# jvstinian/libzombsole

Hardware: AMD Instinct MI355X
Metric: env-steps/sec (whole node), 65 536 parallel 64×64 envs at 1/2/4/8 MI355X (higher is better)
Workload: dtype int32

## Files before the change

### libzombsole_amd/csrc/engine.hip

```cpp
#include <hip/hip_runtime.h>

#include <algorithm>
#include <cstdio>
#include <cstring>
#include <string>
#include <vector>

#include "zs_launch.hpp"
#include "zs_obs_state.hpp"
#include "zs_snapshot.hpp"
#include "zs_record.hpp"
#include "zs_mask.hpp"
#include "zs_entity_obs.hpp"
#include "zs_entity_act.hpp"
#include "zs_autopilot.hpp"
#include "zs_episode.hpp"

static thread_local std::string g_err;

static int fail(int code, const std::string& msg) {
    g_err = msg;
    return code;
}

// ... 10 lines not shown
    do {                                                                                       \
        hipError_t _e = (x);                                                                   \
        if (_e != hipSuccess) return fail(ZS_EHIP, std::string(#x ": ") + hipGetErrorString(_e)); \
    } while (0)

#define TRY(x)             \
    do {                   \
        int _r = (x);      \
        if (_r) return _r; \
    } while (0)

static int launched(const char* name, hipError_t e) {
    return e == hipSuccess ? ZS_OK : fail(ZS_EHIP, std::string(name) + ": " + hipGetErrorString(e));
}
#define LAUNCHCHK(name, x) TRY(launched((name), (x)))

struct zs_handle {
    zs_config cfg;
    zs_launch ov;
    int device;
    Dev d;
    ObsPlan obs;
    StepPlan step;
    struct GraphSet {
        hipGraphExec_t g[2] = {nullptr, nullptr};
        const void* key[9] = {};
        uint64_t used = 0;
    };
    static const int kGraphSets = 4;
    GraphSet gsets[kGraphSets];
    uint64_t gclock = 0;
    bool graphs_stale = false;
    uint64_t* d_gstep = nullptr;
    int graph_pol = 0;
    int reset_side = 0;
    hipStream_t s_reset = nullptr;
    hipEvent_t ev_rfork = nullptr, ev_rjoin = nullptr;
    int state_words;
    std::vector<void*> allocs;
    int32_t* d_state;
    uint64_t* d_seedbuf;
    int* d_err;
    int* d_rlist[2];
    int* d_rcount;
    int rpar = 0;
    uint64_t snap_fp = 0;
    int32_t* d_envp_owner = nullptr;
    void* mask_bound = nullptr;
    int32_t* d_obj_xy = nullptr;
    void* ent_bound = nullptr;
    int ent_kz = 0, ent_kp = 0;
    const int32_t* eact_ids = nullptr;
    void* eact_mask = nullptr;
    int eact_kz = 0, eact_kp = 0;
    NavPlan nav{};
    void* nav_bound = nullptr;
    int nav_fields = 0, nav_max_dist = 0;
    const uint8_t* pilot_policy = nullptr;
    int32_t* pilot_out = nullptr;
    const char* step_last = "";
    EpisodeArgs ep{};
    uint8_t* d_ep_reset = nullptr;
    RenderArgs rn{};
    HostLayout hl{};
    int32_t* h_hin = nullptr;
    int32_t* d_hin = nullptr;
    int32_t* h_hrec = nullptr;
// ... 495 lines not shown
    std::vector<uint64_t> seeds(N);
    for (size_t i = 0; i < N; i++) seeds[i] = i;
    TRY(seed_envs(h, 0, (int)N, seeds.data(), nullptr));
    hipError_t se = hipDeviceSynchronize();
    if (se != hipSuccess) return fail(ZS_EHIP, std::string("zs_create sync: ") + hipGetErrorString(se));
    *out = h;
    owner.h = nullptr;
    return ZS_OK;
}

extern "C" int zs_obs_shape(const zs_handle* h, int32_t out[4]) {
    if (!h || !out) return fail(ZS_EINVAL, "null argument");
    const Dev& d = h->d;
    bool world = d.obs_scope == ZS_OBS_WORLD;
    out[0] = world ? 1 : (d.reward_mode == ZS_REWARD_MULTI ? d.A : 1);
    out[1] = d.obs_enc == ZS_ENC_CHANNELS ? 3 : 1;
    out[2] = world ? d.H : d.obs_w;
    out[3] = world ? d.W : d.obs_w;
    return ZS_OK;
}

extern "C" int zs_seed(zs_handle* h, int32_t env0, int32_t n, const uint64_t* seeds_host, void* stream) {
    if (!h || !seeds_host) return fail(ZS_EINVAL, "null argument");
    NOT_ON_VIEWER(h, "zs_seed");
    return seed_envs(h, env0, n, seeds_host, stream);
}

static int seed_envs(zs_handle* h, int32_t env0, int32_t n, const uint64_t* seeds_host, void* stream) {
    if (env0 < 0 || n < 0 || env0 + n > h->d.N) return fail(ZS_EINVAL, "env range out of bounds");
    if (n == 0) return ZS_OK;
    ENTER(h, stream, s);
    HIPCHK(hipMemcpyAsync(h->d_seedbuf, seeds_host, sizeof(uint64_t) * n, hipMemcpyHostToDevice, s));
    HIPCHK(launch_seed(s, h->d, env0, n, h->d_seedbuf));
    HIPCHK(hipStreamSynchronize(s));
    return ZS_OK;
}

struct TickUnit {
    decltype(&launch_tick_g1) launch;
    decltype(&stamps_g1) stamps;
};
static const TickUnit& tick_unit(int G) {
#define ZS_UNIT(g) {launch_tick_g##g, stamps_g##g}
    static const TickUnit units[7] = {ZS_UNIT(1), ZS_UNIT(2), ZS_UNIT(4), ZS_UNIT(8), ZS_UNIT(16), ZS_UNIT(32), ZS_UNIT(64)};
#undef ZS_UNIT
    return units[__builtin_ctz((unsigned)G)];
}

static int launch_obs(zs_handle* h, const Dev& d, void* obs, const uint8_t* mask, hipStream_t s, int env0 = 0, int env1 = -1) {
    if (!obs) return ZS_OK;
    if (env1 < 0) env1 = d.N;
    const ObsKernel& k = mask ? h->obs.masked : h->obs.full;
    const ObsLaunch o = {k, obs_grid(k, env1 - env0), obs, mask, env0, env1};
    return timed_launch(h, s, h->ev_obs, "observation launch", [&] { return obs_launch(d.obs_dtype, o, s, d); });
}

static int launch_tick(zs_handle* h, const Dev& d, const int32_t* actions, double* rew, uint8_t* done, uint8_t* trunc,
                       uint8_t* listed, uint8_t* reset_out, int* rlist, int* rcount, void* obs, hipStream_t s,
                       int env0 = 0, int env1 = -1) {
    const StepPlan& sp = h->step;
    const int ne = 64 / sp.G;
    if (env1 < 0) env1 = d.N;
    unsigned grid = (unsigned)((env1 - env0 + ne - 1) / ne);
    const int p = h->rpar;
    const TickArgs a = {actions, rew,  done, trunc,      listed,        reset_out,       rlist,   rcount,
                        obs,     env0, env1, sp.n_reset, h->d_rlist[p], h->d_rcount + p, h->d_err};
// ... 31 lines not shown
        }
    }
    if (h->ep.run) HIPCHK(launch_episode_clear(s, h->ep, env_mask_dev, 1));
    if (h->rn.body_col) HIPCHK(launch_render_track(s, h->rn, env_mask_dev, 1));
    return launch_obs(h, h->d, obs_dev, env_mask_dev, s);
}

extern "C" int zs_reset(zs_handle* h, const uint8_t* env_mask_dev, void* obs_dev, void* stream) {
    if (!h) return fail(ZS_EINVAL, "null handle");
    NOT_ON_VIEWER(h, "zs_reset");
    ENTER(h, stream, s);
    TRY(queue_reset(h, env_mask_dev, obs_dev, s));
    int err;
    TRY(read_error_word(h, s, &err));
    return reset_result(err);
}

extern "C" int zs_observe(zs_handle* h, const uint8_t* env_mask_dev, void* obs_dev, void* stream) {
    if (!h || !obs_dev) return fail(ZS_EINVAL, "null argument");
    ENTER(h, stream, s);
    return launch_obs(h, h->d, obs_dev, env_mask_dev, s);
}

extern "C" int zs_step(zs_handle* h, const int32_t* actions_dev, void* obs_dev, double* rewards_dev, uint8_t* done_dev,
                       uint8_t* trunc_dev, uint8_t* listed_dev, uint8_t* reset_dev, void* stream) {
    if (!h || !actions_dev || !rewards_dev || !done_dev || !trunc_dev) return fail(ZS_EINVAL, "null argument");
    NOT_ON_VIEWER(h, "zs_step");
    ENTER(h, stream, s);
    if ((h->ep.run || h->rn.body_col) && !reset_dev) reset_dev = h->d_ep_reset;
    if (h->eact_ids)
        LAUNCHCHK("k_entity_act_decode",
                  launch_entity_act_decode(s, h->d, h->eact_kz, h->eact_kp, nullptr, h->eact_ids, const_cast<int32_t*>(actions_dev)));
    int q = 1 - h->rpar, rc = ZS_OK;
    bool side = false;
    if (!h->step.fused) {
        side = h->reset_side != 0;
        hipStream_t rs = s;
        if (side) {
            HIPCHK(hipEventRecord(h->ev_rfork, s));
            HIPCHK(hipStreamWaitEvent(h->s_reset, h->ev_rfork, 0));
            rs = h->s_reset;
        }
        if (h->graph_pol && side)
            HIPCHK(launch_gen_actions_ctr(s, h->d, (const uint64_t*)h->d_gstep, h->graph_pol, (int32_t*)actions_dev));
        TRY(launch_reset(h, h->d, 1, nullptr, h->d.fobs ? obs_dev : nullptr, rs));
        if (side) HIPCHK(hipEventRecord(h->ev_rjoin, h->s_reset));
    }
    Dev d = h->d;
    d.pol_n = side ? 0 : h->graph_pol;
    d.pol_step = side ? nullptr : h->d_gstep;
    const int p = h->rpar;
    TRY(launch_tick(h, d, actions_dev, rewards_dev, done_dev, trunc_dev, listed_dev, reset_dev, h->d_rlist[q],
                    h->d_rcount + q, obs_dev, s));
    h->rpar = q;
    auto tail_on_error = [&](int code) {
        hipStreamCaptureStatus cs = hipStreamCaptureStatusNone;
        if (hipStreamIsCapturing(s, &cs) == hipSuccess && cs == hipStreamCaptureStatusNone) {
            (void)hipMemsetAsync(h->d_rcount + p, 0, sizeof(int), s);
            if (h->d.defer_respawn) (void)hipMemsetAsync(h->d.resp_count, 0, sizeof(int), s);
        }
        return code;
    };
    if (h->d.defer_respawn) {
        rc = launch_respawn(h, d, s);
        if (rc) return tail_on_error(rc);
    }
    if (side && hipStreamWaitEvent(s, h->ev_rjoin, 0) != hipSuccess) return tail_on_error(fail(ZS_EHIP, "hipStreamWaitEvent"));
    d.tail_cnt0 = h->d_rcount + p;
    d.tail_cnt1 = d.defer_respawn ? d.resp_count : nullptr;
    d.tail_step = h->graph_pol ? h->d_gstep : nullptr;
    if (d.fobs || !obs_dev) {
        rc = launched("k_tail", launch_tail(s, d));
        if (rc) return tail_on_error(rc);
        h->step_last = "k_tail";
    } else {
        rc = launch_obs(h, d, obs_dev, nullptr, s);
        if (rc) return tail_on_error(rc);
        h->step_last = obs_kernel_name(h->obs.full.kind);
    }
    if (h->mask_bound) LAUNCHCHK("k_action_mask", launch_action_mask(s, d, nullptr, h->mask_bound));
    if (h->ent_bound) {
        const EntityArgs g = {h->ent_kz, h->ent_kp, d.nobj, h->d_obj_xy};
        LAUNCHCHK("k_entity_obs", launch_entity_obs(s, d, g, nullptr, h->ent_bound));
    }
    if (h->eact_mask) LAUNCHCHK("k_entity_act_mask", launch_entity_act_mask(s, d, h->eact_kz, h->eact_kp, nullptr, h->eact_mask));
    if (h->nav_bound) {
// ... 260 lines not shown
extern "C" int zs_step_graph_n(zs_handle* h, uint64_t step0, int32_t n_discrete, int32_t n_steps, int32_t* actions_dev,
                               void* obs_dev, double* rewards_dev, uint8_t* done_dev, uint8_t* trunc_dev,
                               uint8_t* listed_dev, uint8_t* reset_dev, void* stream) {
    if (!h || !actions_dev || !rewards_dev || !done_dev || !trunc_dev) return fail(ZS_EINVAL, "null argument");
    NOT_ON_VIEWER(h, "zs_step_graph");
    if (n_discrete < 0 || n_discrete > 7) return fail(ZS_EINVAL, "n_discrete must be in 0..7");
    if (n_steps < 1 || n_steps > 64) return fail(ZS_EINVAL, "n_steps must be in 1..64");
    if (n_discrete != 0 && h->eact_ids)
        return fail(ZS_EINVAL, "zs_step_graph: n_discrete must be 0 while entity-action ids are bound (the generated policy "
                               "would overwrite the decoded rows)");
    ENTER(h, stream, s);
    if (h->graphs_stale) {
        HIPCHK(hipStreamSynchronize(s));
        for (auto& gs : h->gsets) {
            HIPCHK(destroy_graphs(gs));
            gs.used = 0;
        }
        h->graphs_stale = false;
    }
    const void* key[9] = {actions_dev, obs_dev, rewards_dev, done_dev, trunc_dev, listed_dev, reset_dev,
                          (const void*)(intptr_t)n_discrete, (const void*)(intptr_t)n_steps};
    zs_handle::GraphSet* set = nullptr;
    for (auto& gs : h->gsets) {
        bool same = gs.g[0] && gs.g[1];
        for (int k = 0; k < 9 && same; k++) same = key[k] == gs.key[k];
        if (same) set = &gs;
    }
    if (!set) {
        set = &h->gsets[0];
        for (auto& gs : h->gsets)
            if (gs.used < set->used) set = &gs;
        HIPCHK(destroy_graphs(*set));
        if (!h->d_gstep) {
            TRY(dalloc(h, &h->d_gstep, 2));
        }
        uint64_t init[2] = {step0, 0};
        if (n_discrete > 0) HIPCHK(hipMemcpyAsync(h->d_gstep, init, sizeof(init), hipMemcpyHostToDevice, s));
        HIPCHK(hipStreamSynchronize(s));
        hipStream_t cs;
        HIPCHK(hipStreamCreateWithFlags(&cs, hipStreamNonBlocking));
        const int prof = h->prof;
        h->prof = 0;
        const int p0 = h->rpar;
        int rc = ZS_OK;
        for (int g = 0; g < 2 && rc == ZS_OK; g++) {
            hipGraph_t graph = nullptr;
            h->rpar = (p0 + g) & 1;
            if (hipStreamBeginCapture(cs, hipStreamCaptureModeThreadLocal) != hipSuccess) {
                rc = fail(ZS_EHIP, "hipStreamBeginCapture failed");
                break;
            }
            h->graph_pol = n_discrete;
            for (int k = 0; k < n_steps && rc == ZS_OK; k++)
                rc = zs_step(h, actions_dev, obs_dev, rewards_dev, done_dev, trunc_dev, listed_dev, reset_dev, cs);
            h->graph_pol = 0;
            hipError_t ce = hipStreamEndCapture(cs, &graph);
            if (rc == ZS_OK && ce != hipSuccess) rc = fail(ZS_EHIP, std::string("hipStreamEndCapture: ") + hipGetErrorString(ce));
            if (rc == ZS_OK) {
                hipError_t ie = hipGraphInstantiate(&set->g[(p0 + g) & 1], graph, nullptr, nullptr, 0);
                if (ie != hipSuccess) rc = fail(ZS_EHIP, std::string("hipGraphInstantiate: ") + hipGetErrorString(ie));
            }
            if (graph) (void)hipGraphDestroy(graph);
        }
        h->rpar = p0;
        h->prof = prof;
        (void)hipStreamDestroy(cs);
        if (rc != ZS_OK) {
            (void)destroy_graphs(*set);
            return rc;
        }
// ... 296 lines not shown

extern "C" int zs_profile_read(zs_handle* h, double* out) {
    if (!h || !out) return fail(ZS_EINVAL, "null argument");
    HIPCHK(hipSetDevice(h->device));
    double tot[4] = {0.0, 0.0, 0.0, 0.0};
    EventList* lists[4] = {&h->ev_tick, &h->ev_obs, &h->ev_reset, &h->ev_respawn};
    for (int k = 0; k < 4; k++)
        for (auto& pr : *lists[k]) {
            HIPCHK(hipEventSynchronize(h->ev_pool[pr.second]));
            float ms = 0.f;
            HIPCHK(hipEventElapsedTime(&ms, h->ev_pool[pr.first], h->ev_pool[pr.second]));
            tot[k] += ms;
        }
    for (int k = 0; k < 4; k++) out[2 * k] = tot[k], out[2 * k + 1] = (double)lists[k]->size();
    prof_clear(h);
    return ZS_OK;
}

extern "C" int zs_describe(zs_handle* h, char* buf, int32_t len) {
    if (!h || !buf || len <= 0) return fail(ZS_EINVAL, "null argument");
    const Dev& d = h->d;
    const ObsKernel& kf = h->obs.full;
    const StepPlan& p = h->step;
    snprintf(buf, (size_t)len,
             "{\"envs\": %d, \"entities\": %d, \"lanes_per_env\": %d, \"step_kernel\": \"%s\", \"step_lds\": %d, "
             "\"step_wgs_per_cu\": %d, \"rng_window\": %d, \"obs_kernel\": \"%s\", \"reset_side_stream\": %d, "
             "\"reset_lds\": %d, \"respawn\": \"%s\", \"tick_waves\": %d, \"rng_step\": %d, \"par_exec\": %d, "
             "\"obs_kernel_masked\": \"%s\", \"obs_encoders\": \"%s\", \"mask_kernel\": \"k_action_mask\", "
             "\"mask_grid\": %u, \"mask_block\": %d, \"mask_bound\": %d, \"env_params\": %d, \"episode_stats\": %d, "
             "\"render\": %d, \"render_grid\": %d, \"render_block\": %d, \"entity_obs_bound\": %d, \"entity_kz\": %d, "
             "\"entity_kp\": %d, \"autopilot_kernel\": \"k_autopilot\", \"autopilot_grid\": %u, \"autopilot_block\": %d, "
             "\"autopilot_bound\": %d, \"nav_bound\": %d, \"nav_fields\": %d, \"nav_max_dist\": %d, \"nav_kernel\": \"k_nav\", "
             "\"nav_envs_per_wg\": %d, \"nav_block\": %d, \"nav_lds_bytes\": %d, \"entity_act_kernel\": \"k_entity_act\", "
             "\"entity_act_ids_bound\": %d, \"entity_act_mask_bound\": %d, \"step_tail_launch\": \"%s\"}",
             d.N, d.E, p.G, p.fused ? "k_step" : "k_tick", p.lds, p.resident, p.rw_cap,
             d.fobs ? "step launch" : obs_kernel_name(kf.kind), h->reset_side,
             p.reset_lds, p.defer_respawn ? "k_respawn" : "tick", p.tick_waves, p.rw_step,
             d.par_exec, obs_kernel_name(h->obs.masked.kind), obs_encoders_name(kf), zs_mask_grid(d.N), ZS_MASK_BLOCK,
             h->mask_bound ? 1 : 0, (d.flags & ZS_FLAG_ENV_PARAMS) ? 1 : 0, h->ep.run ? 1 : 0, h->rn.body_col ? 1 : 0,
             h->rn.body_col ? h->rn.plan.bands : 0, h->rn.body_col ? ZS_RENDER_BLOCK : 0,
             h->ent_bound ? 1 : 0, h->ent_kz, h->ent_kp, zs_pilot_grid(d.N), ZS_PILOT_BLOCK, h->pilot_out ? 1 : 0,
             h->nav_bound ? 1 : 0, h->nav_fields, h->nav_max_dist, h->nav.envs_per_wg, h->nav.block, h->nav.lds_bytes,
             h->eact_ids ? 1 : 0, h->eact_mask ? 1 : 0, h->step_last);
    return ZS_OK;
}

static int read_log(zs_handle* h, const int32_t* log, const int32_t* log_n, int words, int lo, int32_t env, int32_t* out_host,
                    int32_t cap, int32_t* n_out, void* stream) {
    if (!h || !n_out || (cap > 0 && !out_host)) return fail(ZS_EINVAL, "null argument");
    if (!log) return fail(ZS_EINVAL, "the handle was created without ZS_FLAG_DEATH_LOG");
    if (env < 0 || env >= h->d.N) return fail(ZS_EINVAL, "env out of range");
    ENTER(h, stream, s);
    int32_t n = 0;
    HIPCHK(hipMemcpyAsync(&n, log_n + env, sizeof(int32_t), hipMemcpyDeviceToHost, s));
    HIPCHK(hipStreamSynchronize(s));
    n = std::max(lo, std::min(n, h->d.E));
    const int k = std::min(n < 0 ? -1 - n : n, std::max(0, (int)cap));
    if (k > 0) {
        HIPCHK(hipMemcpyAsync(out_host, log + (size_t)env * h->d.E * words, sizeof(int32_t) * words * k, hipMemcpyDeviceToHost, s));
        HIPCHK(hipStreamSynchronize(s));
    }
    *n_out = n;
    return ZS_OK;
}

extern "C" int zs_action_log(zs_handle* h, int32_t env, int32_t* out_host, int32_t cap, int32_t* n_out, void* stream) {
    return read_log(h, h ? h->d.alog : nullptr, h ? h->d.alog_n : nullptr, 2, h ? -1 - h->d.E : 0, env, out_host, cap, n_out, stream);
}

extern "C" int zs_death_log(zs_handle* h, int32_t env, int32_t* out_host, int32_t cap, int32_t* n_out, void* stream) {
    return read_log(h, h ? h->d.dlog : nullptr, h ? h->d.dlog_n : nullptr, 5, 0, env, out_host, cap, n_out, stream);
}

static int obs_bytes_per_env(const zs_handle* h) {
    int32_t shp[4];
    zs_obs_shape(h, shp);
// ... 178 lines not shown
```

### libzombsole_amd/csrc/zs_device.hpp

```cpp
#pragma once
#include <hip/hip_runtime.h>
#include <stdint.h>

#include "../../include/zombsole_mi355x.h"
#include "zs_obs_plan.hpp"
#include "zs_step_plan.hpp"

#ifndef ZS_RESET_WAVES
#define ZS_RESET_WAVES 3
#endif

#define ZS_MT_M 397
#define ZS_RING_WORDS (2 * ZS_MT_N)

#define EIX(d, s, e) ((size_t)(e) * (d).E + (s))

enum {
    S_T = 0,
    S_DEATHS,
    S_ZD,
    S_EPSTEPS,
    S_NORDER,
    S_NEEDRESET,
    S_PREVZD,
// ... 32 lines not shown
    const int32_t* zspawn;
    const int32_t* agent_weapons;
    const int32_t* agent_codes;
    const int32_t* bot_types;
    int32_t* pos;
    int32_t* life;
    uint8_t* weapon;
    uint8_t* present;
    uint32_t* serial;
    uint8_t* order;
    int32_t* scal;
    int32_t* prev_life;
    uint8_t* listed;
    int32_t* obst_hp;
    uint32_t* hp_dirty;
    const int32_t* hp_init;
    int hp_chunk;
    uint32_t hp_chunk_m;
    uint32_t hp_chunk_m32;
    uint32_t* dead_dirty;
    const uint32_t* dead_zero;
    int dead_chunk;
    uint32_t dead_chunk_m;
    uint32_t dead_chunk_m32;
    const uint32_t* opres_full;
    uint32_t w_m;
    uint32_t* obst_present;
    uint32_t* obst_nonpos;
    uint32_t* dead;
    uint32_t* ring;
    uint32_t* rngst;
    const uint64_t* pol_step;
    int pol_n;
    int* tail_cnt0;
    int* tail_cnt1;
    uint64_t* tail_step;
    uint64_t* seeds;
    int32_t* cand;
    int* resp_list;
    int* resp_count;
    int32_t* dlog;
    int32_t* dlog_n;
    int32_t* alog;
    int32_t* alog_n;
    uint32_t* ovf;
};

#define SC_OBST_MASK 0xffffu
#define SC_KIND_SHIFT 16
#define SC_OBJ_BIT (1u << 20)
#define OPAD_OBJ 8u

#ifdef ZS_STAMPS
#define ZS_NPHASE 28
#define ZS_STAMP_WGS 65536
#endif

enum { EP_INITIAL = 0, EP_MINIMUM, EP_MAXSTEPS, EP_N };
__host__ __device__ __forceinline__ int32_t* envp_cur(const Dev& d) { return d.scal + (size_t)S_NSCAL * d.N; }
__host__ __device__ __forceinline__ int32_t* envp_next(const Dev& d) { return d.scal + (size_t)(S_NSCAL + EP_N) * d.N; }

__device__ __forceinline__ const Dev* zs_launder_dev(const Dev& d0) {
    typedef const __attribute__((address_space(4))) Dev CDev;
    CDev* dp = (CDev*)__builtin_amdgcn_kernarg_segment_ptr();
    asm volatile("" : "+s"(dp));
#ifdef ZS_CHECK_LAUNDER
    if (dp->N != d0.N || dp->E != d0.E || dp->pos != d0.pos || dp->ring != d0.ring) __builtin_trap();
#else
    (void)d0;
#endif
    return (const Dev*)dp;
}

#define ZS_HP_FLOOR (-2147483647)

__device__ __forceinline__ int32_t hp_store_value(const Dev& d, int64_t v) {
    if (v < -32768) {
        uint32_t f = ZS_OVF_INT16;
        if (v < (int64_t)ZS_HP_FLOOR) {
            v = ZS_HP_FLOOR;
            f |= ZS_OVF_INT32;
        }
        if ((__hip_atomic_load(d.ovf, __ATOMIC_RELAXED, __HIP_MEMORY_SCOPE_AGENT) & f) != f) atomicOr(d.ovf, f);
    }
    return (int32_t)v;
}

__device__ __forceinline__ void step_tail(const Dev& d) {
    if (d.tail_cnt0) *d.tail_cnt0 = 0;
    if (d.tail_cnt1) *d.tail_cnt1 = 0;
    if (d.tail_step) *d.tail_step += 1;
}

__device__ __forceinline__ uint64_t splitmix64(uint64_t x) {
    uint64_t z = x + 0x9E3779B97F4A7C15ull;
    z = (z ^ (z >> 30)) * 0xBF58476D1CE4E5B9ull;
    z = (z ^ (z >> 27)) * 0x94D049BB133111EBull;
    return z ^ (z >> 31);
}

static __constant__ int32_t c_discrete[7][3] = {{ZS_ACT_MOVE, 0, 1},  {ZS_ACT_MOVE, -1, 0},       {ZS_ACT_MOVE, 0, -1},
                                         {ZS_ACT_MOVE, 1, 0},  {ZS_ACT_ATTACK_CLOSEST, 0, 0}, {ZS_ACT_HEAL, 0, 0},
                                         {ZS_ACT_HEAL_CLOSEST, 0, 0}};

__device__ __forceinline__ int policy_id(uint64_t seed, uint64_t step, int n, int a) {
    return (int)(splitmix64(splitmix64(splitmix64(seed) ^ step) ^ (uint64_t)a) % (uint64_t)n);
}
__device__ __forceinline__ int32_t policy_action(uint64_t seed, uint64_t step, int n, int k) {
    const int a = k / 3;
    return c_discrete[policy_id(seed, step, n, a)][k - 3 * a];
}

__device__ __forceinline__ int32_t pack_xy(int x, int y) { return (int32_t)((uint32_t)(x & 0xffff) | ((uint32_t)y << 16)); }
__device__ __forceinline__ int unpack_x(int32_t p) { return (int)(int16_t)(p & 0xffff); }
__device__ __forceinline__ int unpack_y(int32_t p) { return (int)(p >> 16); }

__device__ __forceinline__ void wave_sync() {
    __builtin_amdgcn_fence(__ATOMIC_RELEASE, "wavefront");
    __builtin_amdgcn_wave_barrier();
    __builtin_amdgcn_fence(__ATOMIC_ACQUIRE, "wavefront");
}

__device__ __forceinline__ uint32_t mt_temper(uint32_t y) {
    y ^= (y >> 11);
    y ^= (y << 7) & 0x9d2c5680u;
    y ^= (y << 15) & 0xefc60000u;
    y ^= (y >> 18);
    return y;
}

__device__ __forceinline__ uint32_t mt_f(uint32_t a, uint32_t b, uint32_t c) {
    uint32_t y = (a & 0x80000000u) | (b & 0x7fffffffu);
    return c ^ (y >> 1) ^ ((y & 1u) ? 0x9908b0dfu : 0u);
}

__device__ inline void mt_twist_serial(uint32_t* dst, const uint32_t* src) {
    for (int i = 0; i < ZS_MT_N; i++) {
        uint32_t b = (i + 1 < ZS_MT_N) ? src[i + 1] : dst[0];
        uint32_t c = (i + ZS_MT_M < ZS_MT_N) ? src[i + ZS_MT_M] : dst[i + ZS_MT_M - ZS_MT_N];
        dst[i] = mt_f(src[i], b, c);
    }
}

// ... 102 lines not shown
```

### libzombsole_amd/csrc/zs_obs.hpp

```cpp
#pragma once
#include "zs_device.hpp"
#include "zs_obs_plan.hpp"

typedef unsigned int zs_v4u __attribute__((ext_vector_type(4)));
typedef unsigned int zs_v2u __attribute__((ext_vector_type(2)));
typedef int zs_v2i __attribute__((ext_vector_type(2)));
typedef int zs_v4i __attribute__((ext_vector_type(4)));

__device__ __forceinline__ int xcd_remap(int b, int nb) {
    const int q = nb >> 3, r = nb & 7, x = b & 7, k = b >> 3;
    return x * q + (x < r ? x : r) + k;
}

struct XcdDeal {
    int base, span, off, w, ucount;
    __device__ XcdDeal(int b, int nb, int n_units, int W) : w(W) {
        const int q = nb >> 3, r = nb & 7, x = b & 7, j = b >> 3;
        const int gs = x * q + (x < r ? x : r), gx = q + (x < r);
        const int r0 = (int)((long long)n_units * gs / nb), r1 = (int)((long long)n_units * (gs + gx) / nb);
        base = r0;
        span = gx * W;
        off = j * W;
        const int m = r1 - r0 - off;
        ucount = m <= 0 ? 0 : (m / span) * W + min(m % span, W);
// ... 946 lines not shown
    lv4u* st4 = (lv4u*)smem;
    lu8* slots = (lu8*)(smem + stat_bytes + RING_ENC * enc_bytes);
    ZS_LDS int* state = (ZS_LDS int*)(slots + US * SLOT);
    if (threadIdx.x < RING_SLOTS) state[threadIdx.x] = 0;
    if (PATCHED) {
        patch_stage_static(d, smem);
    } else {
        obs_stage_static4(d, st4, threadIdx.x, blockDim.x);
        __syncthreads();
    }
    const int G = gridDim.x, n_units = (env1 - env0 + PAIR - 1) / PAIR;
    const XcdDeal deal(blockIdx.x, G, n_units, RING_WRT);
    const int ucount = deal.ucount;
    auto unit_of = [&](int u) { return deal.unit(u); };
    const int count = ucount ? PAIR * (ucount - 1) + min(PAIR, env1 - env0 - PAIR * unit_of(ucount - 1)) : 0;
    auto unit_env = [&](int u) { return env0 + PAIR * unit_of(u); };
    if (wave >= RING_ENC) {
        for (int u = wave - RING_ENC; u < ucount; u += RING_WRT) {
            const int q = u % US, e = unit_env(u);
            const bool whole = PAIR * u + PAIR <= count;
            for (int h = 0; h < PAIR; h++)
                if (PAIR * u + h < count) ring_wait(&state[PAIR * q + h], 2 * u + 1);
            if (whole) obs_stage_flush<T, NOBS * PAIR, RING_THR>(slots + q * SLOT, out + (size_t)e * BLK, lane);
            else obs_stage_flush<T, NOBS, RING_THR>(slots + q * SLOT, out + (size_t)e * BLK, lane);
            for (int h = 0; h < PAIR; h++) ring_state_store(&state[PAIR * q + h], 2 * u + 2);
        }
        return;
    }
    lu8* img = (lu8*)(smem + stat_bytes + wave * enc_bytes);
    PatchEnc<S> pe(d, smem, img, lane);
    const li32* pos = (const li32*)(img + L.off_pos);
    const int code_s = lane < d.A ? d.agent_codes[lane < d.A ? lane : 0] : (lane < d.A + d.P ? ZS_THING_PLAYER : ZS_THING_ZOMBIE);
    auto item_env = [&](int t) { return unit_env(t / PAIR) + t % PAIR; };
    int t = wave;
    if (t >= count) return;
    auto encode = [&](int t, ObsPrefetch& f, zs_v2u& dq) {
        const Dev& d = *zs_launder_dev(d0);
        const int u = t / PAIR, h = t % PAIR, e = item_env(t);
        if (PATCHED) pe.build(d, f);
        else obs_build_compact(d, L, img, f, code_s, lane);
        const int tn = t + 2 * RING_ENC, tq = t + 4 * RING_ENC;
        obs_prefetch_env(d, item_env(tn < count ? tn : wave), dq, f);
        dq = obs_dirty(d, item_env(tq < count ? tq : wave));
        wave_sync();
        if (!PATCHED) obs_window_compact<NOBS>(d, L, img, lane);
        const int q = u % US;
        if (u >= US) ring_wait(&state[PAIR * q + h], 2 * (u - US) + 2);
        wave_sync();
        ZS_LDS S* ot0 = (ZS_LDS S*)(slots + q * SLOT) + (int)((uintptr_t)(out + (size_t)(e - h) * BLK) & 15) / TS + h * BLK;
#pragma unroll
        for (int a = 0; a < NOBS; a++) {
            if (PATCHED) {
                pe.block(d, ot0 + a * 3 * PLANE, a);
            } else {
                const int32_t ap = pos[a];
                const int ox = unpack_x(ap) - WW / 2, oy = unpack_y(ap) - WW / 2;
                const lu8* wm = img + a * PLANE;
                obs_encode_block<S>(d, L, st4, img, wm, ox, oy, ot0 + a * 3 * PLANE, lane);
            }
        }
        ring_state_store(&state[PAIR * q + h], 2 * u + 1);
    };
    auto envc = [&](int tt) { return item_env(tt < count ? tt : wave); };
    ObsPrefetch fa, fb;
    zs_v2u qa, qb;
    obs_prefetch_env(d, envc(t), OBS_OWN_ROWS, fa);
    obs_prefetch_env(d, envc(t + RING_ENC), obs_dirty(d, envc(t + RING_ENC)), fb);
    qa = obs_dirty(d, envc(t + 2 * RING_ENC));
    qb = obs_dirty(d, envc(t + 3 * RING_ENC));
    for (; t < count; t += 2 * RING_ENC) {
        encode(t, fa, qa);
        if (t + RING_ENC < count) encode(t + RING_ENC, fb, qb);
    }
}

#ifndef BRING_THR
#define BRING_THR RING_THR
#endif
__device__ __forceinline__ uint32_t chunk_of(uint32_t x, uint32_t m32) { return m32 ? __umulhi(x, m32) : x; }


template <typename T, int NOBS>
__global__ void __launch_bounds__(64 * (BRING_ENC + BRING_WRT), 1) k_obs_pbring(Dev d, T* out, int env0, int env1, int us) {
    if (blockIdx.x == 0 && threadIdx.x == 0) step_tail(d);
    extern __shared__ __align__(16) uint8_t smem[];
    typedef typename obs_stage<T>::type S;
    constexpr int WW = 21, PLANE = WW * WW, PER = PLANE / 63, TS = (int)sizeof(T);
    static_assert(PLANE % 63 == 0, "63 lanes x PER rows of three");
    constexpr int PAIR = ring_pair(TS, NOBS), SLOT = obs_stage_slot_bytes(TS, NOBS * PAIR), BLK = NOBS * 3 * PLANE;
    const int wave = __builtin_amdgcn_readfirstlane(threadIdx.x >> 6), lane = threadIdx.x & 63;
    const int encb = pbring_enc_bytes(d.DW, d.OW);
    lv4u* st4 = (lv4u*)smem;
    lu8* slots = (lu8*)(smem + 16 * d.DW + BRING_ENC * encb);
    ZS_LDS int* state = (ZS_LDS int*)(slots + us * SLOT);
    if (threadIdx.x < 8) state[threadIdx.x] = 0;
    obs_stage_static4(d, st4, threadIdx.x, blockDim.x);
    __syncthreads();
    const int G = gridDim.x, n_units = (env1 - env0 + PAIR - 1) / PAIR;
    const XcdDeal deal(blockIdx.x, G, n_units, BRING_WRT);
    const int ucount = deal.ucount;
    const int count = ucount ? PAIR * (ucount - 1) + min(PAIR, env1 - env0 - PAIR * deal.unit(ucount - 1)) : 0;
    auto unit_env = [&](int u) { return env0 + PAIR * deal.unit(u); };
    if (wave >= BRING_ENC) {
        for (int u = wave - BRING_ENC; u < ucount; u += BRING_WRT) {
            const int q = u % us, e = unit_env(u);
            const bool whole = PAIR * u + PAIR <= count;
            for (int h = 0; h < PAIR; h++)
                if (PAIR * u + h < count) ring_wait(&state[PAIR * q + h], 2 * u + 1);
            if (whole) obs_stage_flush<T, NOBS * PAIR, BRING_THR>(slots + q * SLOT, out + (size_t)e * BLK, lane);
            else obs_stage_flush<T, NOBS, BRING_THR>(slots + q * SLOT, out + (size_t)e * BLK, lane);
            for (int h = 0; h < PAIR; h++) ring_state_store(&state[PAIR * q + h], 2 * u + 2);
        }
        return;
    }
    lu32* idead = (lu32*)(smem + 16 * d.DW + wave * encb);
    lu32* iopres = (lu32*)(smem + 16 * d.DW + wave * encb + ((d.DW * 4 + 15) / 16) * 16);
    const int code_s = lane < d.A ? d.agent_codes[lane < d.A ? lane : 0] : (lane < d.A + d.P ? ZS_THING_PLAYER : ZS_THING_ZOMBIE);
    const int W = d.W, H = d.H, sl = lane < d.E ? lane : d.E - 1;
    const int lr = lane / WW, lq = lane - lr * WW;
    auto item_env = [&](int t) { return unit_env(t / PAIR) + t % PAIR; };
    if (wave >= count) return;
    struct R1 {
        int32_t p, l, w, r;
        uint32_t hd, dd;
    };
    struct R23 {
        uint32_t dv[BRING_D], ov[BRING_O];
        int32_t hv[NOBS][PER];
    };
    auto envc = [&](int t) { return item_env(t < count ? t : wave); };
    auto round1 = [&](int t, R1& r) {
        const int e = envc(t);
        r.p = d.pos[EIX(d, sl, e)];
        r.l = d.life[EIX(d, sl, e)];
        r.w = d.weapon[EIX(d, sl, e)];
        r.r = d.present[EIX(d, sl, e)];
        r.hd = d.hp_dirty[e];
        r.dd = d.dead_dirty[e];
    };
    auto round23 = [&](int t, const R1& r, R23& q) {
        const int e = envc(t);
        const uint32_t* dr = d.dead + (size_t)e * d.DW;
#pragma unroll
        for (int i = 0; i < BRING_D; i++) {
            const int w = min(lane + 64 * i, d.DW - 1);
            q.dv[i] = (((r.dd >> chunk_of((uint32_t)w, d.dead_chunk_m32)) & 1u) ? dr : d.dead_zero)[w];
        }
        const uint32_t* orow = r.hd ? d.obst_present + (size_t)e * d.OW : d.opres_full;
#pragma unroll
        for (int i = 0; i < BRING_O; i++) q.ov[i] = orow[min(lane + 64 * i, max(d.OW - 1, 0))];
        const int32_t* hrow = d.obst_hp + (size_t)e * d.O;
#pragma unroll
        for (int a = 0; a < NOBS; a++) {
            const int32_t ap = __builtin_amdgcn_readlane(r.p, a);
// ... 63 lines not shown
#pragma unroll
            for (int a = 0; a < NOBS; a++) {
                const int32_t ap = __builtin_amdgcn_readlane(r.p, a);
                const int dx = x - (unpack_x(ap) - WW / 2), dy = y - (unpack_y(ap) - WW / 2);
                if ((unsigned)dx < (unsigned)WW && (unsigned)dy < (unsigned)WW) {
                    ZS_LDS S* ot = ot0 + a * 3 * PLANE;
                    const int cc = dy * WW + dx;
                    ot[cc] = (S)code_s;
                    ot[PLANE + cc] = obs_val<S>(r.l);
                    ot[2 * PLANE + cc] = (S)r.w;
                }
            }
        }
        ring_state_store(&state[PAIR * qs + h], 2 * u + 1);
        wave_sync();
    };
    R1 ra, rb;
    R23 qa, qb;
    int t = wave;
    round1(t, ra);
    round1(t + BRING_ENC, rb);
    round23(t, ra, qa);
    auto step = [&](int t, R1& rx, R23& qx, R1& ry, R23& qy) {
        build(qx);
        round23(t + BRING_ENC, ry, qy);
        const R1 cur = rx;
        round1(t + 2 * BRING_ENC, rx);
        encode(t, cur, qx);
    };
    for (; t < count; t += 2 * BRING_ENC) {
        step(t, ra, qa, rb, qb);
        if (t + BRING_ENC < count) step(t + BRING_ENC, rb, qb, ra, qa);
    }
}
```

### libzombsole_amd/csrc/zs_tick.hpp

```cpp
#pragma once
#include "zs_device.hpp"
#include "zs_obs.hpp"

#define NOTHING ((int)0x80000000)

enum { K_NONE = 0, K_MOVE = 1, K_ATTACK = 2, K_HEAL = 3, K_DEFER = 4, K_RAISE = 5 };

#ifdef ZS_STAMPS
static __device__ unsigned long long g_stamp_wg[ZS_STAMP_WGS * ZS_NPHASE];
#define STAMP_DECL unsigned long long _st_prev = 0;
#define STAMP(k)                                                                          \
    do {                                                                                  \
        unsigned long long _t;                                                            \
        asm volatile("s_memtime %0\n\ts_waitcnt lgkmcnt(0)" : "=s"(_t)::"memory");      \
        if ((k) > 0 && threadIdx.x == 0 && blockIdx.x < ZS_STAMP_WGS)                     \
            g_stamp_wg[blockIdx.x * ZS_NPHASE + (k)-1] += _t - _st_prev;                  \
        _st_prev = _t;                                                                    \
    } while (0)
#define SUB_DECL unsigned long long _sub_prev;
#define SUB(k)                                                                            \
    do {                                                                                  \
        unsigned long long _t;                                                            \
        asm volatile("s_memtime %0\n\ts_waitcnt lgkmcnt(0)" : "=s"(_t)::"memory");      \
        if ((k) > 0 && blockIdx.x < ZS_STAMP_WGS && c.g == 0)                             \
// ... 1281 lines not shown
    c.lrank = (lu8*)(smem + L.off_rank);
    c.lkind = (lu8*)(smem + L.off_kind);
    c.lperm = (lu8*)(smem + L.off_perm);
    c.lmoved = (lu8*)(smem + L.off_moved);
    c.lact = (li32*)(smem + L.off_act);
    c.xs = (li32*)(smem + L.off_xs);
    c.lists = (li32*)(smem + L.off_lists);
    if (dp->lists_cap)
        for (int i = lane; i < dp->nps + dp->nzs; i += 64) c.lists[i] = i < dp->nps ? dp->pspawn[i] : dp->zspawn[i - dp->nps];

    STAMP_DECL
    STAMP(0);
    int needs_reset = 0, stepping = 0, n_order = 0;
    uint32_t st0 = 0, st = 0;
    int wlen = 0;
    int32_t vp[4], vl[4];
    uint8_t vw[4], vr[4], vo[4];
    int mval = 0, av = 0;
    uint32_t bmv[8], opw = 0u;
    uint32_t wv[4];
    uint64_t pseed = 0, pstep = 0;
    auto window = [&](uint32_t st_, uint32_t& off, uint32_t& slot, uint32_t& ready) {
        off = st_ & 1023u, slot = (st_ >> 10) & 1u, ready = (st_ >> 11) & 1u;
        if (off >= ZS_MT_N && ready) {
            slot ^= 1u;
            off = 0;
            ready = 0;
        }
        const int maxw = off >= ZS_MT_N ? 0 : (ready ? dp->rw_cap : min(dp->rw_cap, ZS_MT_N - (int)off));
        return min(dp->rw_step, maxw);
    };
    const int nmisc = MISC_N + 2 * A;
    int pmin = 0, pmax = 0;
    if (active) {
        if (dp->pol_n) {
            pseed = dp->seeds[e];
            pstep = *dp->pol_step;
        } else if (A) {
            av = actions[(size_t)e * A * 3 + min(j, 3 * A - 1)];
        }
        needs_reset = dp->scal[S_NEEDRESET * N + e];
        n_order = dp->scal[S_NORDER * N + e];
        st = dp->rngst[e];
#pragma unroll
        for (int u = 0; u < 4; u++) {
            const int s = j + u * G;
            if (s < E) {
                vp[u] = dp->pos[EIX(*dp, s, e)];
                vl[u] = dp->life[EIX(*dp, s, e)];
                vw[u] = dp->weapon[EIX(*dp, s, e)];
                vr[u] = dp->present[EIX(*dp, s, e)];
                vo[u] = dp->order[EIX(*dp, s, e)];
            }
        }
        mval = misc_load(*dp, min(j, nmisc - 1), e);
        opw = dp->obst_present[(size_t)e * dp->OW + min(j, max(dp->OW - 1, 0))];
    }
#pragma unroll
    for (int u = 0; u < 8; u++)
        if (64 * u < dp->DW) bmv[u] = dp->obstbits[min(lane + 64 * u, dp->DW - 1)];
    stepping = active && needs_reset == 0;
    if (active && dp->pol_n) {
        for (int k = j; k < 3 * A; k += G) {
            const int32_t v = policy_action(pseed, pstep, dp->pol_n, k);
            ((int32_t*)actions)[(size_t)e * A * 3 + k] = v;
            if (stepping) LACT(c, k) = v;
        }
    }
#pragma unroll
    for (int u = 0; u < 8; u++)
        if (64 * u < dp->DW && lane + 64 * u < dp->DW) bcast_row<NE>(c.bm, lane + 64 * u, bmv[u]);
    for (int w = 512 + lane; w < dp->DW; w += 64) bcast_row<NE>(c.bm, w, dp->obstbits[w]);
    if (stepping) {
#pragma unroll
        for (int u = 0; u < 4; u++) {
            const int s = j + u * G;
            if (s < E) {
                c.lpos[IX(c, s)] = vp[u];
                c.llife[IX(c, s)] = vl[u];
                c.lweap[IX(c, s)] = vw[u];
                c.lpres[IX(c, s)] = vr[u];
                c.lorder[IX(c, s)] = vo[u];
            }
        }
        if (j < nmisc) MISC(c, j) = mval;
        if (!dp->pol_n) {
            if (j < 3 * A) LACT(c, j) = av;
            for (int k = j + G; k < 3 * A; k += G) LACT(c, k) = actions[(size_t)e * A * 3 + k];
        }
        SX(1);
        {
            auto ix = [&](int s) { return IX(c, s); };

            for (int b = j + 4 * G; b < E; b += 4 * G) {
                int32_t vp[4], vl[4];
                uint8_t vw[4], vr[4], vo[4];
#pragma unroll
// ... 253 lines not shown
            dp->order[EIX(*dp, s, e)] = LO(c, s);
        }
        for (int f = j; f < MISC_N + 2 * A; f += G) misc_store(*dp, f, e, MISC(c, f));
    }
    wave_sync();
    STAMP(6);
    ZS_RELOAD_DEV();
    if (dp->fobs && obs_out) {
        const unsigned long long stepmask = __ballot(stepping && leader);
        lu8* img = (lu8*)(smem + L.off_region);
        lu32* st = dp->obs_stat ? (lu32*)(smem + L.off_region + dp->obsl.bytes) : nullptr;
        if (st && stepmask) obs_stage_static(*dp, st, lane, 64);
        for (int g2 = 0; g2 < NE; g2++) {
            if (!((stepmask >> (g2 * G)) & 1ull)) continue;
            obs_build(*dp, dp->obsl, img, base + g2, [&](int s, int& p, int& lf, int& wp, int& pr) {
                p = c.lpos[s * NE + g2];
                lf = c.llife[s * NE + g2];
                wp = c.lweap[s * NE + g2];
                pr = c.lpres[s * NE + g2];
            });
            obs_stream_any(*dp, dp->obsl, st, img, obs_out, base + g2);
            wave_sync();
        }
    }
    STAMP(7);
#undef ZS_RELOAD_DEV
}

template <int G, int W = ZS_STEP_WAVES, bool EARLY = false>
__global__ void __launch_bounds__(64, W) k_tick(Dev d, const int32_t* actions, double* rew, uint8_t* done_out,
                                             uint8_t* trunc_out, uint8_t* listed_out, uint8_t* reset_out,
                                             int* reset_list, int* reset_count, void* obs_out, int env0, int env1) {
    extern __shared__ __align__(16) uint8_t smem[];
    tick_wg<G, EARLY>(d, xcd_remap(blockIdx.x, gridDim.x), actions, rew, done_out, trunc_out, listed_out, reset_out, reset_list,
               reset_count, obs_out, env0, env1, (lu8*)smem);
}
```

Before: 188.6 million.

## Precompute next-step policy actions inside ring obs kernels and defer reset after tick

When graph-captured random policies run with a side reset stream and ring observation encoders, the obs kernel now also computes the next step's policy actions into a side buffer. The tick kernel reads them, validated by a step stamp, instead of rerunning the policy hash. This removes the separate k_gen_actions_ctr launch. The reset launch also moves after the tick on the side stream so it overlaps the tail. It adds stamp bookkeeping in global memory and a cross-kernel step protocol, which could go stale or race if stamps mismatch, in which case it falls back to recomputing.

```diff
diff --git a/libzombsole_amd/csrc/engine.hip b/libzombsole_amd/csrc/engine.hip
--- a/libzombsole_amd/csrc/engine.hip
+++ b/libzombsole_amd/csrc/engine.hip
@@ -66,7 +66,9 @@
     uint64_t gclock = 0;
     bool graphs_stale = false;
     uint64_t* d_gstep = nullptr;
+    int32_t* d_ahead = nullptr;
     int graph_pol = 0;
+    const char* step_policy = "";
     int reset_side = 0;
     hipStream_t s_reset = nullptr;
     hipEvent_t ev_rfork = nullptr, ev_rjoin = nullptr;
@@ -628,6 +630,7 @@
     ENTER(h, stream, s);
     HIPCHK(hipMemcpyAsync(h->d_seedbuf, seeds_host, sizeof(uint64_t) * n, hipMemcpyHostToDevice, s));
     HIPCHK(launch_seed(s, h->d, env0, n, h->d_seedbuf));
+    if (h->d_gstep) HIPCHK(hipMemsetAsync(h->d_gstep + GS_STAMP, 0, 2 * sizeof(uint64_t), s));
     HIPCHK(hipStreamSynchronize(s));
     return ZS_OK;
 }
@@ -725,7 +728,7 @@
         LAUNCHCHK("k_entity_act_decode",
                   launch_entity_act_decode(s, h->d, h->eact_kz, h->eact_kp, nullptr, h->eact_ids, const_cast<int32_t*>(actions_dev)));
     int q = 1 - h->rpar, rc = ZS_OK;
-    bool side = false;
+    bool side = false, ahead = false;
     if (!h->step.fused) {
         side = h->reset_side != 0;
         hipStream_t rs = s;
@@ -734,17 +737,27 @@
             HIPCHK(hipStreamWaitEvent(h->s_reset, h->ev_rfork, 0));
             rs = h->s_reset;
         }
-        if (h->graph_pol && side)
+        ahead = h->graph_pol && side && obs_dev && !h->d.fobs &&
+                (h->obs.full.kind == OBSK_RING || h->obs.full.kind == OBSK_BRING);
+        if (h->graph_pol && side && !ahead)
             HIPCHK(launch_gen_actions_ctr(s, h->d, (const uint64_t*)h->d_gstep, h->graph_pol, (int32_t*)actions_dev));
-        TRY(launch_reset(h, h->d, 1, nullptr, h->d.fobs ? obs_dev : nullptr, rs));
-        if (side) HIPCHK(hipEventRecord(h->ev_rjoin, h->s_reset));
+        if (!ahead) {
+            TRY(launch_reset(h, h->d, 1, nullptr, h->d.fobs ? obs_dev : nullptr, rs));
+            if (side) HIPCHK(hipEventRecord(h->ev_rjoin, h->s_reset));
+        }
     }
     Dev d = h->d;
-    d.pol_n = side ? 0 : h->graph_pol;
-    d.pol_step = side ? nullptr : h->d_gstep;
+    d.pol_n = side && !ahead ? 0 : h->graph_pol;
+    d.pol_step = side && !ahead ? nullptr : h->d_gstep;
+    d.pol_ahead = ahead ? h->d_ahead : nullptr;
+    if (h->graph_pol) h->step_policy = ahead ? "ahead" : side ? "k_gen_actions_ctr" : "step launch";
     const int p = h->rpar;
     TRY(launch_tick(h, d, actions_dev, rewards_dev, done_dev, trunc_dev, listed_dev, reset_dev, h->d_rlist[q],
                     h->d_rcount + q, obs_dev, s));
+    if (ahead) {
+        TRY(launch_reset(h, h->d, 1, nullptr, nullptr, h->s_reset));
+        HIPCHK(hipEventRecord(h->ev_rjoin, h->s_reset));
+    }
     h->rpar = q;
     auto tail_on_error = [&](int code) {
         hipStreamCaptureStatus cs = hipStreamCaptureStatusNone;
@@ -1071,10 +1084,10 @@
             if (gs.used < set->used) set = &gs;
         HIPCHK(destroy_graphs(*set));
         if (!h->d_gstep) {
-            TRY(dalloc(h, &h->d_gstep, 2));
+            TRY(dalloc(h, &h->d_gstep, GS_WORDS));
+            TRY(dalloc(h, &h->d_ahead, (size_t)h->d.N * h->d.A * 3));
         }
-        uint64_t init[2] = {step0, 0};
-        if (n_discrete > 0) HIPCHK(hipMemcpyAsync(h->d_gstep, init, sizeof(init), hipMemcpyHostToDevice, s));
+        if (n_discrete > 0) HIPCHK(hipMemcpyAsync(h->d_gstep + GS_STEP, &step0, sizeof(step0), hipMemcpyHostToDevice, s));
         HIPCHK(hipStreamSynchronize(s));
         hipStream_t cs;
         HIPCHK(hipStreamCreateWithFlags(&cs, hipStreamNonBlocking));
@@ -1437,7 +1450,8 @@
              "\"entity_kp\": %d, \"autopilot_kernel\": \"k_autopilot\", \"autopilot_grid\": %u, \"autopilot_block\": %d, "
              "\"autopilot_bound\": %d, \"nav_bound\": %d, \"nav_fields\": %d, \"nav_max_dist\": %d, \"nav_kernel\": \"k_nav\", "
              "\"nav_envs_per_wg\": %d, \"nav_block\": %d, \"nav_lds_bytes\": %d, \"entity_act_kernel\": \"k_entity_act\", "
-             "\"entity_act_ids_bound\": %d, \"entity_act_mask_bound\": %d, \"step_tail_launch\": \"%s\"}",
+             "\"entity_act_ids_bound\": %d, \"entity_act_mask_bound\": %d, \"step_tail_launch\": \"%s\", "
+             "\"step_policy\": \"%s\"}",
              d.N, d.E, p.G, p.fused ? "k_step" : "k_tick", p.lds, p.resident, p.rw_cap,
              d.fobs ? "step launch" : obs_kernel_name(kf.kind), h->reset_side,
              p.reset_lds, p.defer_respawn ? "k_respawn" : "tick", p.tick_waves, p.rw_step,
@@ -1446,7 +1460,7 @@
              h->rn.body_col ? h->rn.plan.bands : 0, h->rn.body_col ? ZS_RENDER_BLOCK : 0,
              h->ent_bound ? 1 : 0, h->ent_kz, h->ent_kp, zs_pilot_grid(d.N), ZS_PILOT_BLOCK, h->pilot_out ? 1 : 0,
              h->nav_bound ? 1 : 0, h->nav_fields, h->nav_max_dist, h->nav.envs_per_wg, h->nav.block, h->nav.lds_bytes,
-             h->eact_ids ? 1 : 0, h->eact_mask ? 1 : 0, h->step_last);
+             h->eact_ids ? 1 : 0, h->eact_mask ? 1 : 0, h->step_last, h->step_policy);
     return ZS_OK;
 }
 
diff --git a/libzombsole_amd/csrc/zs_device.hpp b/libzombsole_amd/csrc/zs_device.hpp
--- a/libzombsole_amd/csrc/zs_device.hpp
+++ b/libzombsole_amd/csrc/zs_device.hpp
@@ -88,6 +88,7 @@
     uint32_t* rngst;
     const uint64_t* pol_step;
     int pol_n;
+    int32_t* pol_ahead;
     int* tail_cnt0;
     int* tail_cnt1;
     uint64_t* tail_step;
@@ -142,10 +143,19 @@
     return (int32_t)v;
 }
 
+enum { GS_STEP = 0, GS_NEXT, GS_STAMP, GS_STAMP_N, GS_WORDS };
+
 __device__ __forceinline__ void step_tail(const Dev& d) {
     if (d.tail_cnt0) *d.tail_cnt0 = 0;
     if (d.tail_cnt1) *d.tail_cnt1 = 0;
-    if (d.tail_step) *d.tail_step += 1;
+    if (d.tail_step) {
+        const uint64_t t = d.tail_step[GS_STEP] + 1;
+        d.tail_step[GS_STEP] = t;
+        if (d.pol_ahead) {
+            d.tail_step[GS_STAMP] = t;
+            d.tail_step[GS_STAMP_N] = (uint64_t)d.pol_n;
+        }
+    }
 }
 
 __device__ __forceinline__ uint64_t splitmix64(uint64_t x) {
@@ -165,6 +175,20 @@
 __device__ __forceinline__ int32_t policy_action(uint64_t seed, uint64_t step, int n, int k) {
     const int a = k / 3;
     return c_discrete[policy_id(seed, step, n, a)][k - 3 * a];
+}
+
+template <typename F>
+__device__ __forceinline__ void policy_ahead(const Dev& d, int count, int tid, int nthr, F item_env) {
+    const uint64_t step = d.pol_step[GS_NEXT];
+    const int A = d.A, n = d.pol_n;
+    for (int i = tid; i < count * A; i += nthr) {
+        const int t = i / A, a = i - t * A, e = item_env(t);
+        const int id = policy_id(d.seeds[e], step, n, a);
+        int32_t* o = d.pol_ahead + ((size_t)e * A + a) * 3;
+        o[0] = c_discrete[id][0];
+        o[1] = c_discrete[id][1];
+        o[2] = c_discrete[id][2];
+    }
 }
 
 __device__ __forceinline__ int32_t pack_xy(int x, int y) { return (int32_t)((uint32_t)(x & 0xffff) | ((uint32_t)y << 16)); }
diff --git a/libzombsole_amd/csrc/zs_obs.hpp b/libzombsole_amd/csrc/zs_obs.hpp
--- a/libzombsole_amd/csrc/zs_obs.hpp
+++ b/libzombsole_amd/csrc/zs_obs.hpp
@@ -1002,8 +1002,12 @@
     const li32* pos = (const li32*)(img + L.off_pos);
     const int code_s = lane < d.A ? d.agent_codes[lane < d.A ? lane : 0] : (lane < d.A + d.P ? ZS_THING_PLAYER : ZS_THING_ZOMBIE);
     auto item_env = [&](int t) { return unit_env(t / PAIR) + t % PAIR; };
+    auto ahead = [&] {
+        const Dev& d = *zs_launder_dev(d0);
+        if (d.pol_ahead) policy_ahead(d, count, 64 * wave + lane, 64 * RING_ENC, item_env);
+    };
     int t = wave;
-    if (t >= count) return;
+    if (t >= count) return ahead();
     auto encode = [&](int t, ObsPrefetch& f, zs_v2u& dq) {
         const Dev& d = *zs_launder_dev(d0);
         const int u = t / PAIR, h = t % PAIR, e = item_env(t);
@@ -1042,6 +1046,7 @@
         encode(t, fa, qa);
         if (t + RING_ENC < count) encode(t + RING_ENC, fb, qb);
     }
+    ahead();
 }
 
 #ifndef BRING_THR
@@ -1089,7 +1094,10 @@
     const int W = d.W, H = d.H, sl = lane < d.E ? lane : d.E - 1;
     const int lr = lane / WW, lq = lane - lr * WW;
     auto item_env = [&](int t) { return unit_env(t / PAIR) + t % PAIR; };
-    if (wave >= count) return;
+    auto ahead = [&] {
+        if (d.pol_ahead) policy_ahead(d, count, 64 * wave + lane, 64 * BRING_ENC, item_env);
+    };
+    if (wave >= count) return ahead();
     struct R1 {
         int32_t p, l, w, r;
         uint32_t hd, dd;
@@ -1219,4 +1227,5 @@
         step(t, ra, qa, rb, qb);
         if (t + BRING_ENC < count) step(t + BRING_ENC, rb, qb, ra, qa);
     }
-}
+    ahead();
+}
diff --git a/libzombsole_amd/csrc/zs_tick.hpp b/libzombsole_amd/csrc/zs_tick.hpp
--- a/libzombsole_amd/csrc/zs_tick.hpp
+++ b/libzombsole_amd/csrc/zs_tick.hpp
@@ -1337,13 +1337,15 @@
     };
     const int nmisc = MISC_N + 2 * A;
     int pmin = 0, pmax = 0;
+    const int32_t* asrc = dp->pol_ahead ? dp->pol_ahead : actions;
+    uint64_t stamp = 0, stamp_n = 0;
+    if (dp->pol_n) {
+        pstep = dp->pol_step[GS_STEP];
+        if (dp->pol_ahead) stamp = dp->pol_step[GS_STAMP], stamp_n = dp->pol_step[GS_STAMP_N];
+    }
     if (active) {
-        if (dp->pol_n) {
-            pseed = dp->seeds[e];
-            pstep = *dp->pol_step;
-        } else if (A) {
-            av = actions[(size_t)e * A * 3 + min(j, 3 * A - 1)];
-        }
+        if (dp->pol_n) pseed = dp->seeds[e];
+        if (A && (!dp->pol_n || dp->pol_ahead)) av = asrc[(size_t)e * A * 3 + min(j, 3 * A - 1)];
         needs_reset = dp->scal[S_NEEDRESET * N + e];
         n_order = dp->scal[S_NORDER * N + e];
         st = dp->rngst[e];
@@ -1365,9 +1367,10 @@
     for (int u = 0; u < 8; u++)
         if (64 * u < dp->DW) bmv[u] = dp->obstbits[min(lane + 64 * u, dp->DW - 1)];
     stepping = active && needs_reset == 0;
+    const bool ahead = dp->pol_ahead && __builtin_amdgcn_readfirstlane(stamp == pstep && stamp_n == (uint64_t)dp->pol_n);
     if (active && dp->pol_n) {
         for (int k = j; k < 3 * A; k += G) {
-            const int32_t v = policy_action(pseed, pstep, dp->pol_n, k);
+            const int32_t v = ahead ? (k == j ? av : asrc[(size_t)e * A * 3 + k]) : policy_action(pseed, pstep, dp->pol_n, k);
             ((int32_t*)actions)[(size_t)e * A * 3 + k] = v;
             if (stepping) LACT(c, k) = v;
         }
@@ -1687,6 +1690,7 @@
                                              uint8_t* trunc_out, uint8_t* listed_out, uint8_t* reset_out,
                                              int* reset_list, int* reset_count, void* obs_out, int env0, int env1) {
     extern __shared__ __align__(16) uint8_t smem[];
+    if (d.pol_ahead && blockIdx.x == 0 && threadIdx.x == 0) const_cast<uint64_t*>(d.pol_step)[GS_NEXT] = d.pol_step[GS_STEP] + 1;
     tick_wg<G, EARLY>(d, xcd_remap(blockIdx.x, gridDim.x), actions, rew, done_out, trunc_out, listed_out, reset_out, reset_list,
                reset_count, obs_out, env0, env1, (lu8*)smem);
 }
```

Measured after the change: 191.6 million, median of 6. +1.6%, better.
